# TorchIO-project/torchio

Measured on NVIDIA H100. Metric: augmented voxels/sec on 256^3 fp32 Compose pipeline, higher is better.
Workload: dtype f32

## Files before the change

### include/tio_b200.h

```cpp
#ifndef TIO_B200_H
#define TIO_B200_H

#include <stddef.h>
#include <stdint.h>

#ifdef __cplusplus
extern "C" {
#endif

#define TIO_ABI_VERSION 2

enum tio_dtype {
  TIO_F32 = 0,
  TIO_U8 = 1,
  TIO_I8 = 2,
  TIO_I16 = 3,
  TIO_I32 = 4,
  TIO_I64 = 5,
  TIO_F16 = 6,
  TIO_BF16 = 7,
  TIO_F64 = 8
};

enum tio_interp { TIO_NEAREST = 0, TIO_LINEAR = 1, TIO_LABEL_PV = 2 };
// ... 22 lines not shown

int tio_crop_patches(const void* src, void* dst, int elem_bytes, int C, int I, int J, int K,
                     int n, const int32_t* corners, int pi, int pj, int pk, void* stream);

int tio_remap(const void* src, void* dst, int elem_bytes, int B, int C, int I, int J, int K,
              int OI, int OJ, int OK, int off_i, int off_j, int off_k, int mode,
              const void* fill, const uint8_t* flip, void* stream);

int tio_upload(const void* host_pinned, void* dst_device, size_t bytes, void* stream);

int tio_min_sample0(const float* src, int C, int64_t n, float* fill, void* stream);

int tio_blur(const float* src, float* dst, float* scratch,
             int B, int C, int I, int J, int K,
             const float* taps, const int32_t* radius, int R, int axes_mask,
             const uint8_t* identity, void* stream);

size_t tio_mt19937_table_bytes(void);
int tio_mt19937_build_table(void* host_blob, size_t bytes);
size_t tio_randn_mt19937_workspace_bytes(uint64_t offset, uint64_t n);
int tio_randn_mt19937(uint64_t seed, uint64_t offset, uint64_t n, float* z,
                      const void* table, void* workspace, size_t workspace_bytes,
                      void* stream);

int tio_moments(const float* src, const uint8_t* mask, int64_t n, double* out3, void* stream);
size_t tio_quantiles_workspace_bytes(void);
int tio_quantiles(const float* src, const uint8_t* mask, int64_t n, const double* q_host, int m,
                  float* values, double* weights, double* count, void* workspace,
                  size_t workspace_bytes, void* stream);
int tio_rescale(const float* src, float* dst, int B, int64_t per_elem, float lo, float hi,
                const float* sub, const float* div, const float* mul, const float* add,
                const uint8_t* keep, int flags, void* stream);

size_t tio_quantiles_batched_workspace_bytes(int B, int m);
int tio_quantiles_batched(const void* src, int dtype, const uint8_t* mask, int B, int64_t per_elem,
                          const double* q_host, int m, float* values, double* weights, double* count,
                          uint8_t* has_nan, void* workspace, size_t workspace_bytes, void* stream);
int tio_histogram_tables(const float* values, const double* weights, const uint8_t* has_nan,
                         const float* landmarks, int B, int m, float* tables, void* stream);
int tio_histogram_map(const void* src, void* dst, int dtype, int B, int64_t per_elem,
                      const float* tables, int m, void* stream);

int tio_intensity_fused(const float* src, float* dst, float* scratch,
                        int B, int C, int I, int J, int K,
                        const float* coarse, int si, int sj, int sk,
                        const uint8_t* bias_identity, int bias_divide,
// ... 51 lines not shown
```

### torchio_b200/_native.py

```python

from __future__ import annotations

import ctypes
from ctypes import c_char_p, c_float, c_int, c_int64, c_size_t, c_uint64, c_void_p
from pathlib import Path

LIB_PATH = Path(__file__).resolve().parent / "csrc" / "libtio_b200.so"

_SIGNATURES = {
    "tio_abi_version": [],
    "tio_resample": [c_void_p, c_void_p, c_int] + [c_int] * 8
    + [c_void_p, c_void_p, c_void_p] + [c_int] * 3
    + [c_void_p, c_void_p, c_int, c_int, c_void_p, c_int, c_void_p, c_size_t, c_void_p],
    "tio_resample_workspace_bytes": [c_int, c_int, c_int, c_int],
    "tio_min_sample0": [c_void_p, c_int, c_int64, c_void_p, c_void_p],
    "tio_upload": [c_void_p, c_void_p, c_size_t, c_void_p],
    "tio_remap": [c_void_p, c_void_p, c_int] + [c_int] * 8 + [c_int] * 3 + [c_int, c_void_p, c_void_p, c_void_p],
    "tio_crop_patches": [c_void_p, c_void_p, c_int] + [c_int] * 5 + [c_void_p, c_int, c_int, c_int, c_void_p],
    "tio_blur": [c_void_p, c_void_p, c_void_p] + [c_int] * 5
    + [c_void_p, c_void_p, c_int, c_int, c_void_p, c_void_p],
    "tio_moments": [c_void_p, c_void_p, c_int64, c_void_p, c_void_p],
    "tio_quantiles_workspace_bytes": [],
    "tio_quantiles": [c_void_p, c_void_p, c_int64, c_void_p, c_int, c_void_p, c_void_p, c_void_p, c_void_p,
                      c_size_t, c_void_p],
    "tio_quantiles_batched_workspace_bytes": [c_int, c_int],
    "tio_quantiles_batched": [c_void_p, c_int, c_void_p, c_int, c_int64, c_void_p, c_int, c_void_p, c_void_p,
                              c_void_p, c_void_p, c_void_p, c_size_t, c_void_p],
    "tio_histogram_tables": [c_void_p, c_void_p, c_void_p, c_void_p, c_int, c_int, c_void_p, c_void_p],
    "tio_histogram_map": [c_void_p, c_void_p, c_int, c_int, c_int64, c_void_p, c_int, c_void_p],
    "tio_rescale": [c_void_p, c_void_p, c_int, c_int64, c_float, c_float, c_void_p, c_void_p, c_void_p, c_void_p,
                    c_void_p, c_int, c_void_p],
    "tio_onehot": [c_void_p, c_int, c_int, c_int64, c_void_p, c_int, c_void_p, c_void_p],
    "tio_label_argmax": [c_void_p, c_int, c_int, c_int64, c_void_p, c_float, c_void_p, c_int, c_void_p],
    "tio_mt19937_table_bytes": [],
    "tio_mt19937_build_table": [c_void_p, c_size_t],
    "tio_randn_mt19937_workspace_bytes": [c_uint64, c_uint64],
    "tio_randn_mt19937": [c_uint64, c_uint64, c_uint64, c_void_p, c_void_p, c_void_p, c_size_t,
                          c_void_p],
    "tio_intensity_fused": [c_void_p, c_void_p, c_void_p] + [c_int] * 5
    + [c_void_p, c_int, c_int, c_int, c_void_p, c_int]
    + [c_void_p, c_void_p, c_int, c_int]
    + [c_void_p] * 5 + [c_uint64, c_int, c_int, c_void_p, c_void_p],
    "tio_labels_to_image": [c_void_p, c_int, c_int, c_int, c_int64, c_void_p, c_int, c_void_p, c_void_p, c_void_p,
                            c_uint64, c_int, c_void_p, c_void_p],
    "tio_label_lut": [c_void_p, c_void_p, c_int, c_int64, c_void_p, c_void_p, c_int, c_int, c_void_p],
    "tio_label_contour": [c_void_p, c_int, c_int, c_int, c_int, c_int, c_void_p, c_void_p],
    "tio_onehot_classes": [c_void_p, c_int, c_int, c_int, c_int64, c_int, c_void_p, c_void_p],
    "tio_label_range": [c_void_p, c_int, c_int, c_int, c_int64, c_void_p, c_void_p],
    "tio_channel_argmax": [c_void_p, c_int, c_int, c_int, c_int64, c_void_p, c_void_p],
    "tio_interpolate": [c_void_p, c_void_p, c_int, c_int, c_int, c_int, c_int, c_int, c_int, c_int, c_void_p,
                        c_void_p, c_int, c_void_p],
    "tio_axis_resample": [c_void_p, c_void_p, c_int, c_int, c_int, c_int, c_int, c_int, c_void_p, c_void_p,
                          c_void_p, c_void_p, c_int, c_int, c_void_p],
    "tio_clamp": [c_void_p, c_void_p, c_int, c_int, c_int64, c_void_p, c_void_p, c_void_p],
    "tio_mask": [c_void_p, c_int, c_int, c_void_p, c_int, c_void_p, c_int, c_void_p, c_int, c_int, c_int, c_int64,
                 c_void_p, c_void_p],
    "tio_swap_patches": [c_void_p] + [c_int] * 9 + [c_void_p, c_int, c_int, c_void_p, c_void_p, c_void_p],
    "tio_components": [c_void_p] + [c_int] * 6 + [c_void_p, c_int, c_int64, c_int, c_int] + [c_void_p] * 4,
    "tio_component_roots": [c_void_p, c_int, c_int, c_int64] + [c_void_p] * 4,
    "tio_keep_largest": [c_void_p, c_int, c_int, c_int64, c_int, c_void_p, c_int, c_int64, c_int] + [c_void_p] * 5,
}
# ... 35 lines not shown
```

### torchio_b200/csrc/build.py

```python

from __future__ import annotations

import os
import subprocess
import sys
from concurrent.futures import ThreadPoolExecutor
from pathlib import Path

HERE = Path(__file__).resolve().parent
ROOT = HERE.parent.parent
SOURCES = ["error.cu", "resample.cu", "resample_tile.cu", "resample_fast.cu", "upload.cu", "fused_intensity.cu",
           "mt19937_jump.cpp", "mt19937.cu", "patches.cu", "stats.cu", "labels.cu", "labels_to_image.cu",
           "label_maps.cu", "interpolate.cu", "clamp_mask_swap.cu", "components.cu"]
HEADERS = [HERE / "common.cuh", HERE / "resample_common.cuh", HERE / "resample_tile.cuh", HERE / "tma.cuh",
           HERE / "mt19937_layout.h", HERE / "label_lookup.cuh", HERE / "image_dtype.cuh",
           ROOT / "include" / "tio_b200.h",
           Path(__file__).resolve()]
OBJ = HERE / "_obj"
OUT = HERE / "libtio_b200.so"

ARCH = ["-gencode", "arch=compute_90a,code=sm_90a"]
NVCC_FLAGS = [
    *ARCH,
    "-O3", "-std=c++17", "-lineinfo",
    "-Xcompiler", "-fPIC",
    "-Xptxas", "-v",
]


def needs_build() -> bool:
    if not OUT.exists():
        return True
    newest = max(p.stat().st_mtime for p in [*(HERE / s for s in SOURCES), *HEADERS])
    return OUT.stat().st_mtime < newest


def _compile(source: str) -> tuple[str, int, str]:
    src = HERE / source
    obj = OBJ / (Path(source).stem + ".o")
# ... 38 lines not shown
```

### torchio_b200/csrc/fused_intensity.cu

```cuda
#include "common.cuh"
#include "tma.cuh"

namespace tio {

__device__ __forceinline__ float rician(float x, float n1, float n2) {
  float s = __fadd_rn(x, n1);
  return sqrtf(__fadd_rn(__fmul_rn(s, s), __fmul_rn(n2, n2)));
}


__device__ __forceinline__ uint4 philox4x32_10(uint4 ctr, uint2 key) {
  const uint32_t M0 = 0xD2511F53u, M1 = 0xCD9E8D57u, W0 = 0x9E3779B9u, W1 = 0xBB67AE85u;
#pragma unroll
  for (int r = 0; r < 7; ++r) {
    uint32_t hi0 = __umulhi(M0, ctr.x), lo0 = M0 * ctr.x;
    uint32_t hi1 = __umulhi(M1, ctr.z), lo1 = M1 * ctr.z;
    ctr = make_uint4(hi1 ^ ctr.y ^ key.x, lo1, hi0 ^ ctr.w ^ key.y, lo0);
    key.x += W0;
    key.y += W1;
  }
  return ctr;
}

__device__ __forceinline__ void box_muller(uint32_t a, uint32_t b, float& n0, float& n1) {
  float u1 = ((float)(a >> 8) + 0.5f) * (1.0f / 16777216.0f);
  float u2 = ((float)(b >> 8)) * (1.0f / 16777216.0f);
  float rad;
  asm("sqrt.approx.ftz.f32 %0, %1;" : "=f"(rad) : "f"(-2.0f * __logf(u1)));
  float s, c;
  __sincosf(6.283185307179586f * u2, &s, &c);
  n0 = rad * c;
  n1 = rad * s;
}


__device__ __forceinline__ float abs_pow(float ax, float g) {
  float l, p;
  asm("lg2.approx.f32 %0, %1;" : "=f"(l) : "f"(ax));
  asm("ex2.approx.f32 %0, %1;" : "=f"(p) : "f"(__fmul_rn(g, l)));
  return p;
}

__device__ __forceinline__ float signed_pow(float x, float gam) {
  if (gam == 1.0f) return x;
  float ax = fabsf(x);
  float p = abs_pow(ax, gam);
  p = ax == 0.0f ? 0.0f : p;
  return x < 0.0f ? -p : p;
}

constexpr int A_TJ = 32;
constexpr int A_TK = 64;
constexpr int A_PLANES = 16;

struct BiasArgs {
  const float* coarse;
  const uint8_t* identity;
  int si, sj, sk;
  float sc_i, sc_j, sc_k;
  int divide;
};

struct BlurArgs {
  const float* taps;
  const int32_t* radius;
  int R;
};

struct NoiseArgs {
  const float* mean;
  const float* std;
  const uint8_t* keep;
// ... 192 lines not shown
    for (int o = 0; o < 4; ++o) acc[o] = __fmaf_rn(tk[F_R + t], win[F_HK + o + t], acc[o]);
  return make_float4(acc[0], acc[1], acc[2], acc[3]);
}

template <int RJ>
__device__ __forceinline__ void jconv8(const float* __restrict__ Bw, const int jy, const int kx,
                                       const float* tj, float* acc) {
  float win[8 + 2 * RJ];
#pragma unroll
  for (int w = 0; w < 8 + 2 * RJ; ++w) win[w] = Bw[(F_R - RJ + jy + w) * A_TK + kx];
  if (RJ == 0) {
#pragma unroll
    for (int o = 0; o < 8; ++o) acc[o] = win[o];
    return;
  }
#pragma unroll
  for (int o = 0; o < 8; ++o) acc[o] = 0.0f;
#pragma unroll
  for (int t = -RJ; t <= RJ; ++t)
#pragma unroll
    for (int o = 0; o < 8; ++o) acc[o] = __fmaf_rn(tj[F_R + t], win[o + t + RJ], acc[o]);
}

__device__ __forceinline__ float signed_pow_pos(float x, float g) {
  const float p = abs_pow(fabsf(x), g);
  return x < 0.0f ? -p : p;
}

template <bool HAS_EPI>
__global__ void __launch_bounds__(256, 3)
jk6_kernel(const __grid_constant__ CUtensorMap tmap, float* __restrict__ dst, int B, int C, int I,
           int J, int K, BlurArgs bl, NoiseArgs nz, const float* __restrict__ gamma) {
  extern __shared__ __align__(128) float smem[];
  float* Abuf = smem;
  float* Bbuf = smem + 2 * F_ABUF;
  float* taps_s = Bbuf + 2 * F_BBUF;
  uint64_t* bars = reinterpret_cast<uint64_t*>(taps_s + 32);

  const int tiles_i = (I + A_PLANES - 1) / A_PLANES;
  const int bc = blockIdx.z / tiles_i;
  const int i_begin = (blockIdx.z % tiles_i) * A_PLANES;
  const int i_end = min(i_begin + A_PLANES, I);
  const int b = bc / C;
  const int j0 = blockIdx.y * A_TJ, k0 = blockIdx.x * A_TK;
  const int tid = threadIdx.x;
  const int64_t n = (int64_t)I * J * K;

  auto issue = [&](int i, int s) {
    const uint32_t bar = smem_u32(bars + s);
    mbar_expect_tx(bar, (uint32_t)(F_ABUF * sizeof(float)));
    tma_load_3d(smem_u32(Abuf + s * F_ABUF), &tmap, k0 - F_HK, j0 - F_R, bc * I + i, bar);
  };
  if (tid == 0) {
    mbar_init(smem_u32(bars + 0), 1);
    mbar_init(smem_u32(bars + 1), 1);
    mbar_fence_init();
    issue(i_begin, 0);
  }

  const int R = bl.R;
  const int rj = bl.radius[1 * B + b], rk = bl.radius[2 * B + b];
  const bool noise_on = HAS_EPI && nz.mode != 0 && (!nz.keep || nz.keep[b]);
  const float mu = (HAS_EPI && nz.mode) ? nz.mean[b] : 0.0f, sd = (HAS_EPI && nz.mode) ? nz.std[b] : 0.0f;
  const float gam = (HAS_EPI && gamma) ? gamma[b] : 1.0f;
  const int gamma_mode = !(HAS_EPI && gamma) || gam == 1.0f ? 0 : (gam > 0.0f ? 1 : 2);

  if (tid < 2 * (2 * F_R + 1)) {
    const int axis = tid < (2 * F_R + 1) ? 2 : 1;
    const int s = tid < (2 * F_R + 1) ? tid : tid - (2 * F_R + 1);
    const int off = s - F_R, rr = axis == 2 ? rk : rj;
    float v = 0.0f;
    if (rr > 0 && off >= -rr && off <= rr) v = bl.taps[((int64_t)axis * B + b) * (2 * R + 1) + R + off];
    taps_s[(axis == 2 ? 0 : 13) + s] = v;
  }
  __syncthreads();
  float tk[2 * F_R + 1], tj[2 * F_R + 1];
#pragma unroll
  for (int t = 0; t < 2 * F_R + 1; ++t) { tk[t] = taps_s[t]; tj[t] = taps_s[13 + t]; }

  const int row_lo = F_R - rj, row_hi = F_R + A_TJ + rj;
  const int rsrc_lo = max(0, F_R - j0), rsrc_hi = min(F_ROWS - 1, J - 1 - j0 + F_R);
  const int clo = max(0, F_HK - k0), chi = min(F_COLS - 1, K - 1 - k0 + F_HK);
  const bool kfix = (clo > F_HK - rk) || (chi < F_HK + A_TK + rk - 1);

  const int k4 = (tid & 15) * 4;
  const int kx = tid & 63, jy = (tid >> 6) * 8;
  const int k = k0 + kx;
  const int valid = (k < K) ? min(8, J - (j0 + jy)) : 0;
// ... 66 lines not shown
      default: jconv8<6>(Bw, jy, kx, tj, acc); break;
    }
    if (valid > 0) {
      if (HAS_EPI && noise_on) {
        if (nz.mode == 2) {
          const uint2 key = make_uint2((uint32_t)nz.philox_seed, (uint32_t)(nz.philox_seed >> 32));
#pragma unroll
          for (int h = 0; h < 2; ++h) {
            const uint64_t gidx = (uint64_t)(flat0 + (int64_t)(4 * h) * K);
            uint4 rr = philox4x32_10(make_uint4((uint32_t)gidx, (uint32_t)(gidx >> 32), 0u, 0x6a6bu), key);
            box_muller(rr.x, rr.y, z1[4 * h], z1[4 * h + 1]);
            box_muller(rr.z, rr.w, z1[4 * h + 2], z1[4 * h + 3]);
            if (nz.rician) {
              uint4 r2 = philox4x32_10(make_uint4((uint32_t)gidx, (uint32_t)(gidx >> 32), 1u, 0x6a6bu), key);
              box_muller(r2.x, r2.y, z2[4 * h], z2[4 * h + 1]);
              box_muller(r2.z, r2.w, z2[4 * h + 2], z2[4 * h + 3]);
            }
          }
        }
        if (nz.rician) {
#pragma unroll
          for (int o = 0; o < 8; ++o)
            acc[o] = rician(acc[o], __fadd_rn(mu, __fmul_rn(sd, z1[o])), __fadd_rn(mu, __fmul_rn(sd, z2[o])));
        } else {
#pragma unroll
          for (int o = 0; o < 8; ++o) acc[o] = __fadd_rn(acc[o], __fadd_rn(mu, __fmul_rn(sd, z1[o])));
        }
      }
      if (gamma_mode == 1) {
#pragma unroll
        for (int o = 0; o < 8; ++o) acc[o] = signed_pow_pos(acc[o], gam);
      } else if (gamma_mode == 2) {
#pragma unroll
        for (int o = 0; o < 8; ++o) acc[o] = signed_pow(acc[o], gam);
      }
      float* yp = dst + flat0;
      if (valid == 8) {
#pragma unroll
        for (int o = 0; o < 8; ++o, yp += K) *yp = acc[o];
      } else {
#pragma unroll
        for (int o = 0; o < 8; ++o, yp += K)
          if (o < valid) *yp = acc[o];
      }
    }
    __syncthreads();
  }
}

template <int V, bool HAS_BIAS>
__global__ void __launch_bounds__(256)
march_kernel(const float* __restrict__ src, float* __restrict__ dst, int B, int C, int I, int J,
             int K, BlurArgs bl, BiasArgs bi, NoiseArgs nz, const float* __restrict__ gamma) {
  extern __shared__ __align__(16) float smem[];
  const int bc = blockIdx.z;
  const int b = bc / C;
  const int tid = threadIdx.y * blockDim.x + threadIdx.x;
  const int k = (blockIdx.x * blockDim.x + threadIdx.x) * V;
// ... 175 lines not shown
  const int64_t n = (int64_t)I * J * K;
  const float* x = src + (int64_t)bc * n;
  float* y = dst + (int64_t)bc * n;

  const int r = bl.taps ? bl.radius[0 * B + b] : 0;
  float* tapi = smem;
  float* g = smem + 16;
  const int ns = HAS_BIAS ? bi.si * bi.sj * bi.sk : 0;
  const bool bias_on = HAS_BIAS && !(bi.identity && bi.identity[b]);
  if (tid < W) {
    const int off = tid - F_R;
    tapi[tid] = (r > 0 && off >= -r && off <= r) ? bl.taps[((int64_t)0 * B + b) * (2 * bl.R + 1) + bl.R + off] : 0.0f;
  }
  if (bias_on) {
    const float* gs = bi.coarse + (int64_t)bc * ns;
    for (int t = tid; t < ns; t += 256) g[t] = gs[t];
  }
  __syncthreads();
  if (k >= K || j >= J) return;

  const bool noise_on = EPI && nz.mode != 0 && (!nz.keep || nz.keep[b]);
  const float mu = (EPI && nz.mode) ? nz.mean[b] : 0.0f, sd = (EPI && nz.mode) ? nz.std[b] : 0.0f;
  const float gam = (EPI && gamma) ? gamma[b] : 1.0f;
  const int gamma_mode = !(EPI && gamma) || gam == 1.0f ? 0 : (gam > 0.0f ? 1 : 2);

  LerpAxis lj, lk[4];
  int o00[4], o01[4], o10[4], o11[4];
  int cur0 = -1, cur1 = -1;
  float r_lo[4], r_hi[4];
  if (bias_on) {
    lj = lerp_axis(bi.sc_j, bi.sj, j);
#pragma unroll
    for (int v = 0; v < 4; ++v) {
      lk[v] = lerp_axis(bi.sc_k, bi.sk, k + v);
      o00[v] = lj.i0 * bi.sk + lk[v].i0; o01[v] = lj.i0 * bi.sk + lk[v].i1;
      o10[v] = lj.i1 * bi.sk + lk[v].i0; o11[v] = lj.i1 * bi.sk + lk[v].i1;
    }
  }
  const int col = j * K + k;
  const int plane = J * K;

  float4* fifo = reinterpret_cast<float4*>(g + ((ns + 3) / 4) * 4) + tid;
  auto fifo_issue = [&](int pl) {
    if (pl < I) {
      const uint32_t sa = (uint32_t)__cvta_generic_to_shared(fifo + (pl & (M6_PF - 1)) * 256);
      asm volatile("cp.async.cg.shared.global [%0], [%1], 16;" ::"r"(sa), "l"(x + (int64_t)pl * plane + col) : "memory");
    }
// ... 11 lines not shown
      const LerpAxis li = lerp_axis(bi.sc_i, bi.si, i);
      if (li.i0 != cur0 || li.i1 != cur1) {
        const float* p0 = g + (li.i0 * bi.sj) * bi.sk;
        const float* p1 = g + (li.i1 * bi.sj) * bi.sk;
#pragma unroll
        for (int v = 0; v < 4; ++v) {
          const float a0 = lerp2(lk[v].l0, p0[o00[v]], lk[v].l1, p0[o01[v]]);
          const float a1 = lerp2(lk[v].l0, p0[o10[v]], lk[v].l1, p0[o11[v]]);
          r_lo[v] = lerp2(lj.l0, a0, lj.l1, a1);
          const float b0 = lerp2(lk[v].l0, p1[o00[v]], lk[v].l1, p1[o01[v]]);
          const float b1 = lerp2(lk[v].l0, p1[o10[v]], lk[v].l1, p1[o11[v]]);
          r_hi[v] = lerp2(lj.l0, b0, lj.l1, b1);
        }
        cur0 = li.i0; cur1 = li.i1;
      }
#pragma unroll
      for (int v = 0; v < 4; ++v) {
        const float f = expf(lerp2(li.l0, r_lo[v], li.l1, r_hi[v]));
        out[v] = bi.divide ? __fdiv_rn(out[v], f) : __fmul_rn(out[v], f);
      }
    }
  };

  auto finish = [&](int i, float* v) {
    const int64_t o = (int64_t)i * plane + col;
    if (EPI) {
      if (noise_on) {
        const int64_t flat = (int64_t)bc * n + o;
        float z1[4], z2[4];
        if (nz.mode == 1) {
          const float4 t = __ldcs((const float4*)(nz.z + flat));
          z1[0] = t.x; z1[1] = t.y; z1[2] = t.z; z1[3] = t.w;
          if (nz.rician) {
            const float4 u = __ldcs((const float4*)(nz.z2 + flat));
            z2[0] = u.x; z2[1] = u.y; z2[2] = u.z; z2[3] = u.w;
          }
        } else {
          const uint2 key = make_uint2((uint32_t)nz.philox_seed, (uint32_t)(nz.philox_seed >> 32));
          const uint64_t gidx = (uint64_t)(flat / 4);
          uint4 rr = philox4x32_10(make_uint4((uint32_t)gidx, (uint32_t)(gidx >> 32), 0u, 0x5eedu), key);
          box_muller(rr.x, rr.y, z1[0], z1[1]);
          box_muller(rr.z, rr.w, z1[2], z1[3]);
          if (nz.rician) {
            uint4 r2 = philox4x32_10(make_uint4((uint32_t)gidx, (uint32_t)(gidx >> 32), 1u, 0x5eedu), key);
            box_muller(r2.x, r2.y, z2[0], z2[1]);
            box_muller(r2.z, r2.w, z2[2], z2[3]);
          }
        }
#pragma unroll
        for (int q = 0; q < 4; ++q) {
          const float n1 = __fadd_rn(mu, __fmul_rn(sd, z1[q]));
          if (nz.rician) v[q] = rician(v[q], n1, __fadd_rn(mu, __fmul_rn(sd, z2[q])));
          else v[q] = __fadd_rn(v[q], n1);
        }
      }
      if (gamma_mode == 1) {
#pragma unroll
        for (int q = 0; q < 4; ++q) v[q] = signed_pow_pos(v[q], gam);
      } else if (gamma_mode == 2) {
#pragma unroll
        for (int q = 0; q < 4; ++q) v[q] = signed_pow(v[q], gam);
      }
    }
    *(float4*)(y + o) = make_float4(v[0], v[1], v[2], v[3]);
  };

  if (r == 0) {
    for (int i = 0; i < I; ++i) {
      float v[4];
      load_plane(i, v);
      finish(i, v);
    }
    return;
  }

  float tp[W];
#pragma unroll
  for (int t = 0; t < W; ++t) tp[t] = tapi[t];
  float ring[W][4];
  {
    float first[4];
    load_plane(0, first);
#pragma unroll
    for (int sl = 0; sl < W; ++sl)
#pragma unroll
// ... 295 lines not shown
```

### torchio_b200/csrc/mt19937.cu

```cuda
#include "common.cuh"
#include "mt19937_layout.h"

namespace tio {

constexpr int MT_N = 624, MT_M = 397, MT_DEG = 19937;
constexpr int MT_SEQ = MT_DEG + MT_N;
constexpr int MT_OFFS = (MT_SEQ + 7) / 4 * 4;

__device__ __forceinline__ uint32_t mt_twist(uint32_t a, uint32_t b, uint32_t c) {
  const uint32_t y = (a & 0x80000000u) | (b & 0x7fffffffu);
  return c ^ (y >> 1) ^ ((y & 1u) ? 0x9908b0dfu : 0u);
}

__device__ __forceinline__ uint32_t mt_temper(uint32_t y) {
  y ^= y >> 11;
  y ^= (y << 7) & 0x9d2c5680u;
  y ^= (y << 15) & 0xefc60000u;
  y ^= y >> 18;
  return y;
}

__global__ void mt_seed_kernel(uint32_t seed, uint32_t* __restrict__ states) {
  if (threadIdx.x == 0) {
    uint32_t v = seed;
// ... 90 lines not shown
  float sn, cs;
  sincos_0_2pi(theta, sn, cs);
  zc = radius * cs;
  zs = radius * sn;
}

template <int ID, int COUNT>
__device__ __forceinline__ void mt_bar_sync() {
  asm volatile("bar.sync %0, %1;" ::"n"(ID), "n"(COUNT) : "memory");
}
template <int ID, int COUNT>
__device__ __forceinline__ void mt_bar_arrive() {
  asm volatile("bar.arrive %0, %1;" ::"n"(ID), "n"(COUNT) : "memory");
}

constexpr int MT_ROUND = 4;
constexpr int MT_RING = 2 * MT_ROUND;
constexpr int MT_ITEMS = MT_ROUND * MT_N / 8;
constexpr int MT_PRODUCERS = 256;
constexpr int MT_CONSUMERS = (MT_ITEMS + 31) / 32 * 32;
constexpr int MT_THREADS = MT_PRODUCERS + MT_CONSUMERS;
constexpr int MT_BAR_PROD = 1, MT_BAR_FULL = 2, MT_BAR_EMPTY = 4;

__global__ void __launch_bounds__(MT_THREADS, 2)
mt_normal_kernel(const uint32_t* __restrict__ states, int q_first, unsigned long long L,
                 unsigned long long offset, unsigned long long n, float* __restrict__ z) {
  __shared__ __align__(16) uint32_t ring[MT_RING * MT_N];
  const int tid = threadIdx.x;
  const int q = q_first + blockIdx.x;
  const unsigned long long seg_begin = (unsigned long long)q * L;
  const unsigned long long lo = max(seg_begin, offset);
  const unsigned long long hi = min(seg_begin + L, offset + n);
  if (lo >= hi) return;
  const int lo_rel = (int)(lo - seg_begin), hi_rel = (int)(hi - seg_begin);
  const int rounds = ((hi_rel + MT_N - 1) / MT_N + MT_ROUND - 1) / MT_ROUND;
  if (tid < MT_PRODUCERS) {
    constexpr int W = MT_N - MT_M;
    const uint32_t* w = states + (size_t)q * MT_N;
    uint32_t* start = ring + (MT_RING - 1) * MT_N;
    for (int t = tid; t < MT_N; t += MT_PRODUCERS) start[t] = w[t];
    mt_bar_sync<MT_BAR_PROD, MT_PRODUCERS>();
    for (int r = 0; r < rounds; ++r) {
      if (r >= 2) {
        if (r & 1) mt_bar_sync<MT_BAR_EMPTY + 1, MT_THREADS>();
        else mt_bar_sync<MT_BAR_EMPTY, MT_THREADS>();
      }
      for (int i = 0; i < MT_ROUND; ++i) {
        const int b = r * MT_ROUND + i;
        const uint32_t* cur = ring + ((b + MT_RING - 1) % MT_RING) * MT_N;
        uint32_t* nxt = ring + (b % MT_RING) * MT_N;
        if (tid < W) nxt[tid] = mt_twist(cur[tid], cur[tid + 1], cur[tid + MT_M]);
        mt_bar_sync<MT_BAR_PROD, MT_PRODUCERS>();
        if (tid < W) nxt[W + tid] = mt_twist(cur[W + tid], cur[W + tid + 1], nxt[tid]);
        mt_bar_sync<MT_BAR_PROD, MT_PRODUCERS>();
        if (tid < MT_N - 2 * W) {
          const int k = 2 * W + tid;
          const uint32_t c = (k + 1 < MT_N) ? cur[k + 1] : nxt[0];
          nxt[k] = mt_twist(cur[k], c, nxt[k - W]);
        }
        mt_bar_sync<MT_BAR_PROD, MT_PRODUCERS>();
      }
      if (r & 1) mt_bar_arrive<MT_BAR_FULL + 1, MT_THREADS>();
      else mt_bar_arrive<MT_BAR_FULL, MT_THREADS>();
    }
  } else {
    const int c = tid - MT_PRODUCERS;
    const int blk = c / (MT_N / 8), item = c % (MT_N / 8);
    const int word = 16 * (item >> 1) + 4 * (item & 1);
    const long long seg_to_z = (long long)seg_begin - (long long)offset;
    const bool vec = ((reinterpret_cast<uintptr_t>(z) & 15) == 0);
    for (int r = 0; r < rounds; ++r) {
      if (r & 1) mt_bar_sync<MT_BAR_FULL + 1, MT_THREADS>();
      else mt_bar_sync<MT_BAR_FULL, MT_THREADS>();
      const int b = r * MT_ROUND + blk;
      const int group = b * MT_N + (word & ~15);
      if (c < MT_ITEMS && group >= lo_rel && group < hi_rel) {
        const uint32_t* x = ring + (b % MT_RING) * MT_N + word;
        const uint4 a = *reinterpret_cast<const uint4*>(x);
        const uint4 s = *reinterpret_cast<const uint4*>(x + 8);
        float4 zc, zs;
        mt_box_muller(a.x, s.x, zc.x, zs.x);
        mt_box_muller(a.y, s.y, zc.y, zs.y);
        mt_box_muller(a.z, s.z, zc.z, zs.z);
        mt_box_muller(a.w, s.w, zc.w, zs.w);
        float* zp = z + (seg_to_z + b * MT_N + word);
        if (vec) {
          *reinterpret_cast<float4*>(zp) = zc;
          *reinterpret_cast<float4*>(zp + 8) = zs;
        } else {
          zp[0] = zc.x; zp[1] = zc.y; zp[2] = zc.z; zp[3] = zc.w;
          zp[8] = zs.x; zp[9] = zs.y; zp[10] = zs.z; zp[11] = zs.w;
        }
      }
      if (r + 2 < rounds) {
        if (r & 1) mt_bar_arrive<MT_BAR_EMPTY + 1, MT_THREADS>();
        else mt_bar_arrive<MT_BAR_EMPTY, MT_THREADS>();
      }
    }
  }
}

}

using namespace tio;

constexpr uint64_t MT_L = 1ull << tio_mt::kLog2L;

extern "C" size_t tio_randn_mt19937_workspace_bytes(uint64_t offset, uint64_t n) {
  const uint64_t q_hi = (offset + n + MT_L - 1) / MT_L;
  return (size_t)(q_hi + tio_mt::kS1) * MT_N * 4;
}

extern "C" int tio_randn_mt19937(uint64_t seed, uint64_t offset, uint64_t n, float* z,
                                 const void* table, void* workspace, size_t workspace_bytes,
                                 void* stream) {
  TIO_CHECK_ARG(z && table && workspace, "tio_randn_mt19937: null pointer");
  TIO_CHECK_ARG(n >= 16 && (n % 16) == 0 && (offset % 16) == 0,
                "tio_randn_mt19937: n and offset must be multiples of 16 (n >= 16)");
  const int S2 = tio_mt::kS2, S1 = tio_mt::kS1, stride = tio_mt::kStride;
  const uint64_t q_lo = offset / MT_L, q_hi = (offset + n + MT_L - 1) / MT_L;
  TIO_CHECK_ARG(q_hi <= (uint64_t)S1 * S2, "tio_randn_mt19937: stream position beyond %d segments", S1 * S2);
  TIO_CHECK_ARG(workspace_bytes >= tio_randn_mt19937_workspace_bytes(offset, n),
                "tio_randn_mt19937: workspace too small");
  cudaStream_t st = (cudaStream_t)stream;
  uint32_t* states = (uint32_t*)workspace;
  const uint16_t* polys = (const uint16_t*)((const char*)table + tio_mt::kHeaderBytes);
  mt_seed_kernel<<<1, 32, 0, st>>>((uint32_t)seed, states);
  const size_t jump_smem = (size_t)(MT_OFFS + 2048) * 4;
  cudaFuncSetAttribute(mt_jump_kernel, cudaFuncAttributeMaxDynamicSharedMemorySize, (int)jump_smem);
  const int m_lo = (int)(q_lo / S2), m_hi = (int)((q_hi - 1) / S2);
  const int m_first = m_lo > 1 ? m_lo : 1;
  if (m_hi >= m_first) {
    constexpr int kCoarseParts = 8;
    const size_t pitch = (size_t)S2 * MT_N * 4;
    cudaMemset2DAsync(states + (size_t)m_first * S2 * MT_N, pitch, 0, MT_N * 4, m_hi - m_first + 1, st);
    mt_jump_kernel<<<(m_hi - m_first + 1) * kCoarseParts, 640, jump_smem, st>>>(states, polys, stride, m_first,
                                                                             S2, 0, kCoarseParts);
  }
  mt_jump_kernel<<<(unsigned)(q_hi - q_lo), 640, jump_smem, st>>>(states, polys, stride, (int)q_lo, S2, 1, 1);
  mt_normal_kernel<<<(unsigned)(q_hi - q_lo), MT_THREADS, 0, st>>>(states, (int)q_lo, MT_L, offset, n, z);
  TIO_CHECK_LAUNCH();
  return 0;
}
```

### torchio_b200/ops.py

```python

from __future__ import annotations

import os
import threading

import numpy as np
import torch
from torch import Tensor

from . import _native, tables

DTYPE_CODES = {
    torch.float32: 0, torch.uint8: 1, torch.int8: 2,
    torch.int16: 3, torch.int32: 4, torch.int64: 5,
}
NEAREST, LINEAR, LABEL_PV = 0, 1, 2
FLAG_PASSTHROUGH, FLAG_ELASTIC = 1, 2

_counter = threading.local()


def launches() -> int:
    return getattr(_counter, "n", 0)

# ... 460 lines not shown
            table = _mt_device_tables.get(key)
            if table is None:
                table = mt19937_host_table().to(device)
                torch.cuda.synchronize(device)
                _mt_device_tables[key] = table
    return table


def randn_mt19937(seed: int, offset: int, n: int, device, out: Tensor | None = None) -> Tensor:
    device = torch.device(device)
    if n < 16 or n % 16 or offset % 16 or offset + n > MT_MAX_WORDS:
        raise ValueError("randn_mt19937: offset and n must be multiples of 16, n >= 16,"
                         " offset + n <= 2**31")
    z = torch.empty(n, dtype=torch.float32, device=device) if out is None else out
    lib = _native.lib()
    ws_bytes = lib.tio_randn_mt19937_workspace_bytes(offset, n)
    workspace = torch.empty(ws_bytes, dtype=torch.uint8, device=device)
    table = _mt_table(device)
    with torch.cuda.device(device):
        _native.call("tio_randn_mt19937", int(seed) & 0xFFFFFFFF, offset, n, _ptr(z), _ptr(table),
                     _ptr(workspace), ws_bytes, torch.cuda.current_stream(device).cuda_stream)
    _count(4)
    return z



_cuda_rng_lock = threading.Lock()


def labels_to_image(labels: Tensor, label_values, means, stds, draw=None) -> Tensor:
    if labels.dtype not in DTYPE_CODES:
        raise TypeError(f"labels_to_image: unsupported label dtype {labels.dtype}")
    if labels.ndim != 5:
        raise ValueError(f"labels_to_image expects (B, C, I, J, K), got {tuple(labels.shape)}")
    b, c = int(labels.shape[0]), int(labels.shape[1])
    vox = int(np.prod(labels.shape[2:]))
    numel = b * vox
    tables.check_randn_numel(numel)
    _require_cuda(labels, "labels_to_image")
    if torch.cuda.is_current_stream_capturing():
        raise RuntimeError("labels_to_image: CUDA-graph capture is not supported (the generator offsets are"
                           " reserved on the host)")
    values = np.ascontiguousarray(np.asarray(label_values, dtype=np.int64).reshape(-1))
    n = int(values.shape[0])
    if n and np.any(np.diff(values) <= 0):
        raise ValueError("labels_to_image: label_values must be strictly ascending")
# ... 306 lines not shown
```

### torchio_b200/transforms/intensity.py

```python

from __future__ import annotations

import os
import warnings
from typing import Any

import numpy as np
import torch
from torch import Tensor

from .. import ops, tables
from ..data import ImagesBatch, LabelMap, ScalarImage, SubjectsBatch
from ..params import to_nonneg_range, to_range
from .base import IntensityTransform, Transform, chunk_info, staged_derived


def _as_f32(data: Tensor) -> Tensor:
    return data if data.dtype == torch.float32 else data.float()




class BiasField(IntensityTransform):
    def __init__(self, *, std=0.5, scale: float = 0.025, **kwargs: Any) -> None:
# ... 183 lines not shown
        mean = self._mask_identity(self.mean.sample_1d(n), keep, identity=0.0)
        std = self._mask_identity(self.std.sample_1d(n), keep, identity=0.0)
        params = {
            "mean": self._serialize_param(mean), "std": self._serialize_param(std),
            "seed": seed, "rician": self.rician,
        }
        self._tag_batched(params, batch, n, keep, ["mean", "std"])
        return params

    def apply_transform(self, batch: SubjectsBatch, params: dict[str, Any]) -> SubjectsBatch:
        run_stages(self._get_images(batch), [_noise_stage_factory(params)])
        return batch


def _noise_stage_factory(params):
    mode = _noise_mode()
    generator = torch.Generator(device="cpu")
    generator.manual_seed(params["seed"])
    rician = bool(params.get("rician", False))
    keep = params.get("_keep")

    consumed = [0]

    def draw(shape, device):
        n = int(np.prod(shape))
        info = chunk_info()
        if info is None:
            start, n_full = consumed[0], n
        else:
            per = n // shape[0]
            start, n_full = consumed[0] + per * info.b0, per * info.total
        on_device = (not ragged[0] and n >= 16 and n % 16 == 0 and start % 16 == 0
                     and n_full % 16 == 0 and start + n <= ops.MT_MAX_WORDS
                     and device.type == "cuda")
        if info is not None and not on_device:
            raise RuntimeError("Noise: this batch cannot be streamed in slices (ragged normal stream)")
        if n_full < 16 or n_full % 16:
            ragged[0] = True
        consumed[0] += n_full + (16 if (n_full >= 16 and n_full % 16) else 0)
        if on_device:
            return ops.randn_mt19937(params["seed"], start, n, device).view(shape), None
        if host_state[0] != start:
            skip = start - host_state[0]
            if skip % 16 == 0 and skip >= 16:
                torch.randn(skip, generator=generator)
            else:
                raise RuntimeError("Noise: cannot realign the host generator (ragged stream)")
        pin = torch.cuda.is_available()
        z = torch.empty(shape, dtype=torch.float32, pin_memory=pin)
        torch.randn(shape, generator=generator, out=z)
        host_state[0] = consumed[0]
        return None, z

    host_state = [0]
    ragged = [False]

    def stage(ib, index):
        shape = ib.data.shape
        b = shape[0]
        out = {
            "mean": tables.per_element_vector(params["mean"], b),
            "std": tables.per_element_vector(params["std"], b),
            "keep": None if keep is None else np.asarray(keep, dtype=np.uint8),
            "rician": rician,
        }
        if mode == "philox":
            out["noise_mode"] = 2
            out["philox_seed"] = (int(params["seed"]) << 8) | (index & 0xFF)
            return out
        out["noise_mode"] = 1
        z_dev, z_host = draw(shape, ib.data.device)
        out["z" if z_dev is not None else "z_host"] = z_dev if z_dev is not None else z_host
        if rician:
            z_dev, z_host = draw(shape, ib.data.device)
            out["z2" if z_dev is not None else "z2_host"] = z_dev if z_dev is not None else z_host
        return out

    return stage




class Gamma(IntensityTransform):
    def __init__(self, *, log_gamma=0.0, **kwargs: Any) -> None:
        super().__init__(**kwargs)
        self.log_gamma = to_range(log_gamma)
        self._warn_if_noop(is_noop=self.log_gamma.is_constant(0.0), hint="log_gamma=(-0.3, 0.3)")

    @property
    def supports_per_instance_params(self) -> bool:
        return True

    @property
    def supports_per_instance_p(self) -> bool:
        return True

    def supports_chunks(self, batch: SubjectsBatch) -> bool:
        return True
# ... 360 lines not shown
_TABLE_KEYS = ("coarse", "bias_identity", "taps", "radius", "mean", "std", "keep", "gamma")


def run_stages(images, stage_builders) -> None:
    for index, ib in enumerate(images.values()):
        kwargs: dict[str, Any] = {}
        for build in stage_builders:
            stage = build(ib, index)
            if stage:
                kwargs.update(stage)
        if not kwargs:
            continue
        data = ib.data
        device = data.device
        uploaded = ops.upload(device, *[kwargs.get(k) for k in _TABLE_KEYS])
        for key, value in zip(_TABLE_KEYS, uploaded, strict=True):
            if key in kwargs:
                kwargs[key] = value
        z_host, z2_host = kwargs.pop("z_host", None), kwargs.pop("z2_host", None)
        if z_host is not None:
            kwargs["z"] = z_host.to(device, non_blocking=True)
        if z2_host is not None:
            kwargs["z2"] = z2_host.to(device, non_blocking=True)
        out = ops.intensity_fused(_as_f32(data), **kwargs)
        promotes = ("gamma" in kwargs or "mean" in kwargs) and data.dtype != torch.float64
        ib.data = out if promotes or out.dtype == data.dtype else out.to(data.dtype)
```

Measured before the change: 49.40 billion.

## Fuse MT19937 Gaussian noise and gamma into the RNG kernel epilogue

```diff
diff --git a/include/tio_b200.h b/include/tio_b200.h
--- a/include/tio_b200.h
+++ b/include/tio_b200.h
@@ -68,6 +68,11 @@
 int tio_randn_mt19937(uint64_t seed, uint64_t offset, uint64_t n, float* z,
                       const void* table, void* workspace, size_t workspace_bytes,
                       void* stream);
+
+int tio_noise_mt19937(uint64_t seed, uint64_t offset, uint64_t n, const float* src, float* dst,
+                      uint64_t elem_words, const float* mean, const float* std,
+                      const uint8_t* keep, const float* gamma, const void* table,
+                      void* workspace, size_t workspace_bytes, void* stream);
 
 int tio_moments(const float* src, const uint8_t* mask, int64_t n, double* out3, void* stream);
 size_t tio_quantiles_workspace_bytes(void);
diff --git a/torchio_b200/_native.py b/torchio_b200/_native.py
--- a/torchio_b200/_native.py
+++ b/torchio_b200/_native.py
@@ -37,6 +37,8 @@
     "tio_randn_mt19937_workspace_bytes": [c_uint64, c_uint64],
     "tio_randn_mt19937": [c_uint64, c_uint64, c_uint64, c_void_p, c_void_p, c_void_p, c_size_t,
                           c_void_p],
+    "tio_noise_mt19937": [c_uint64, c_uint64, c_uint64, c_void_p, c_void_p, c_uint64, c_void_p, c_void_p,
+                          c_void_p, c_void_p, c_void_p, c_void_p, c_size_t, c_void_p],
     "tio_intensity_fused": [c_void_p, c_void_p, c_void_p] + [c_int] * 5
     + [c_void_p, c_int, c_int, c_int, c_void_p, c_int]
     + [c_void_p, c_void_p, c_int, c_int]
diff --git a/torchio_b200/csrc/build.py b/torchio_b200/csrc/build.py
--- a/torchio_b200/csrc/build.py
+++ b/torchio_b200/csrc/build.py
@@ -14,7 +14,7 @@
            "label_maps.cu", "interpolate.cu", "clamp_mask_swap.cu", "components.cu"]
 HEADERS = [HERE / "common.cuh", HERE / "resample_common.cuh", HERE / "resample_tile.cuh", HERE / "tma.cuh",
            HERE / "mt19937_layout.h", HERE / "label_lookup.cuh", HERE / "image_dtype.cuh",
-           ROOT / "include" / "tio_b200.h",
+           HERE / "intensity_epilogue.cuh", ROOT / "include" / "tio_b200.h",
            Path(__file__).resolve()]
 OBJ = HERE / "_obj"
 OUT = HERE / "libtio_b200.so"
diff --git a/torchio_b200/csrc/fused_intensity.cu b/torchio_b200/csrc/fused_intensity.cu
--- a/torchio_b200/csrc/fused_intensity.cu
+++ b/torchio_b200/csrc/fused_intensity.cu
@@ -1,4 +1,5 @@
 #include "common.cuh"
+#include "intensity_epilogue.cuh"
 #include "tma.cuh"
 
 namespace tio {
@@ -33,21 +34,6 @@
   n1 = rad * s;
 }
 
-
-__device__ __forceinline__ float abs_pow(float ax, float g) {
-  float l, p;
-  asm("lg2.approx.f32 %0, %1;" : "=f"(l) : "f"(ax));
-  asm("ex2.approx.f32 %0, %1;" : "=f"(p) : "f"(__fmul_rn(g, l)));
-  return p;
-}
-
-__device__ __forceinline__ float signed_pow(float x, float gam) {
-  if (gam == 1.0f) return x;
-  float ax = fabsf(x);
-  float p = abs_pow(ax, gam);
-  p = ax == 0.0f ? 0.0f : p;
-  return x < 0.0f ? -p : p;
-}
 
 constexpr int A_TJ = 32;
 constexpr int A_TK = 64;
@@ -286,11 +272,6 @@
     for (int o = 0; o < 8; ++o) acc[o] = __fmaf_rn(tj[F_R + t], win[o + t + RJ], acc[o]);
 }
 
-__device__ __forceinline__ float signed_pow_pos(float x, float g) {
-  const float p = abs_pow(fabsf(x), g);
-  return x < 0.0f ? -p : p;
-}
-
 template <bool HAS_EPI>
 __global__ void __launch_bounds__(256, 3)
 jk6_kernel(const __grid_constant__ CUtensorMap tmap, float* __restrict__ dst, int B, int C, int I,
@@ -327,7 +308,7 @@
   const bool noise_on = HAS_EPI && nz.mode != 0 && (!nz.keep || nz.keep[b]);
   const float mu = (HAS_EPI && nz.mode) ? nz.mean[b] : 0.0f, sd = (HAS_EPI && nz.mode) ? nz.std[b] : 0.0f;
   const float gam = (HAS_EPI && gamma) ? gamma[b] : 1.0f;
-  const int gamma_mode = !(HAS_EPI && gamma) || gam == 1.0f ? 0 : (gam > 0.0f ? 1 : 2);
+  const int gamma_mode = gamma_mode_of(HAS_EPI ? gamma : nullptr, gam);
 
   if (tid < 2 * (2 * F_R + 1)) {
     const int axis = tid < (2 * F_R + 1) ? 2 : 1;
@@ -440,18 +421,9 @@
 #pragma unroll
           for (int o = 0; o < 8; ++o)
             acc[o] = rician(acc[o], __fadd_rn(mu, __fmul_rn(sd, z1[o])), __fadd_rn(mu, __fmul_rn(sd, z2[o])));
-        } else {
-#pragma unroll
-          for (int o = 0; o < 8; ++o) acc[o] = __fadd_rn(acc[o], __fadd_rn(mu, __fmul_rn(sd, z1[o])));
-        }
-      }
-      if (gamma_mode == 1) {
-#pragma unroll
-        for (int o = 0; o < 8; ++o) acc[o] = signed_pow_pos(acc[o], gam);
-      } else if (gamma_mode == 2) {
-#pragma unroll
-        for (int o = 0; o < 8; ++o) acc[o] = signed_pow(acc[o], gam);
-      }
+        }
+      }
+      noise_gamma(acc, z1, HAS_EPI && noise_on && !nz.rician, mu, sd, gamma_mode, gam);
       float* yp = dst + flat0;
       if (valid == 8) {
 #pragma unroll
@@ -673,7 +645,7 @@
   const bool noise_on = EPI && nz.mode != 0 && (!nz.keep || nz.keep[b]);
   const float mu = (EPI && nz.mode) ? nz.mean[b] : 0.0f, sd = (EPI && nz.mode) ? nz.std[b] : 0.0f;
   const float gam = (EPI && gamma) ? gamma[b] : 1.0f;
-  const int gamma_mode = !(EPI && gamma) || gam == 1.0f ? 0 : (gam > 0.0f ? 1 : 2);
+  const int gamma_mode = gamma_mode_of(EPI ? gamma : nullptr, gam);
 
   LerpAxis lj, lk[4];
   int o00[4], o01[4], o10[4], o11[4];
@@ -731,12 +703,12 @@
     }
   };
 
-  auto finish = [&](int i, float* v) {
+  auto finish = [&](int i, float (&v)[4]) {
     const int64_t o = (int64_t)i * plane + col;
     if (EPI) {
+      float z1[4], z2[4];
       if (noise_on) {
         const int64_t flat = (int64_t)bc * n + o;
-        float z1[4], z2[4];
         if (nz.mode == 1) {
           const float4 t = __ldcs((const float4*)(nz.z + flat));
           z1[0] = t.x; z1[1] = t.y; z1[2] = t.z; z1[3] = t.w;
@@ -756,20 +728,13 @@
             box_muller(r2.z, r2.w, z2[2], z2[3]);
           }
         }
-#pragma unroll
-        for (int q = 0; q < 4; ++q) {
-          const float n1 = __fadd_rn(mu, __fmul_rn(sd, z1[q]));
-          if (nz.rician) v[q] = rician(v[q], n1, __fadd_rn(mu, __fmul_rn(sd, z2[q])));
-          else v[q] = __fadd_rn(v[q], n1);
-        }
-      }
-      if (gamma_mode == 1) {
-#pragma unroll
-        for (int q = 0; q < 4; ++q) v[q] = signed_pow_pos(v[q], gam);
-      } else if (gamma_mode == 2) {
-#pragma unroll
-        for (int q = 0; q < 4; ++q) v[q] = signed_pow(v[q], gam);
-      }
+        if (nz.rician) {
+#pragma unroll
+          for (int q = 0; q < 4; ++q)
+            v[q] = rician(v[q], __fadd_rn(mu, __fmul_rn(sd, z1[q])), __fadd_rn(mu, __fmul_rn(sd, z2[q])));
+        }
+      }
+      noise_gamma(v, z1, noise_on && !nz.rician, mu, sd, gamma_mode, gam);
     }
     *(float4*)(y + o) = make_float4(v[0], v[1], v[2], v[3]);
   };
diff --git a/torchio_b200/csrc/intensity_epilogue.cuh b/torchio_b200/csrc/intensity_epilogue.cuh
--- /dev/null
+++ b/torchio_b200/csrc/intensity_epilogue.cuh
@@ -0,0 +1,45 @@
+#pragma once
+
+namespace tio {
+
+__device__ __forceinline__ float abs_pow(float ax, float g) {
+  float l, p;
+  asm("lg2.approx.f32 %0, %1;" : "=f"(l) : "f"(ax));
+  asm("ex2.approx.f32 %0, %1;" : "=f"(p) : "f"(__fmul_rn(g, l)));
+  return p;
+}
+
+__device__ __forceinline__ float signed_pow(float x, float gam) {
+  if (gam == 1.0f) return x;
+  float ax = fabsf(x);
+  float p = abs_pow(ax, gam);
+  p = ax == 0.0f ? 0.0f : p;
+  return x < 0.0f ? -p : p;
+}
+
+__device__ __forceinline__ float signed_pow_pos(float x, float g) {
+  const float p = abs_pow(fabsf(x), g);
+  return x < 0.0f ? -p : p;
+}
+
+__device__ __forceinline__ int gamma_mode_of(const float* gamma, float g) {
+  return !gamma || g == 1.0f ? 0 : (g > 0.0f ? 1 : 2);
+}
+
+template <int N>
+__device__ __forceinline__ void noise_gamma(float (&v)[N], const float (&z)[N], bool noise_on, float mu,
+                                            float sd, int gamma_mode, float g) {
+  if (noise_on) {
+#pragma unroll
+    for (int i = 0; i < N; ++i) v[i] = __fadd_rn(v[i], __fadd_rn(mu, __fmul_rn(sd, z[i])));
+  }
+  if (gamma_mode == 1) {
+#pragma unroll
+    for (int i = 0; i < N; ++i) v[i] = signed_pow_pos(v[i], g);
+  } else if (gamma_mode == 2) {
+#pragma unroll
+    for (int i = 0; i < N; ++i) v[i] = signed_pow(v[i], g);
+  }
+}
+
+}
diff --git a/torchio_b200/csrc/mt19937.cu b/torchio_b200/csrc/mt19937.cu
--- a/torchio_b200/csrc/mt19937.cu
+++ b/torchio_b200/csrc/mt19937.cu
@@ -1,4 +1,5 @@
 #include "common.cuh"
+#include "intensity_epilogue.cuh"
 #include "mt19937_layout.h"
 
 namespace tio {
@@ -136,10 +137,27 @@
 constexpr int MT_THREADS = MT_PRODUCERS + MT_CONSUMERS;
 constexpr int MT_BAR_PROD = 1, MT_BAR_FULL = 2, MT_BAR_EMPTY = 4;
 
+struct MtApply {
+  const float* src;
+  float* dst;
+  uint32_t elem_words;
+  const float* mean;
+  const float* std;
+  const uint8_t* keep;
+  const float* gamma;
+};
+
+__device__ __forceinline__ void mt_cp_async16(void* smem, const void* gmem) {
+  const uint32_t sa = (uint32_t)__cvta_generic_to_shared(smem);
+  asm volatile("cp.async.cg.shared.global [%0], [%1], 16;" ::"r"(sa), "l"(gmem) : "memory");
+}
+
+template <bool APPLY>
 __global__ void __launch_bounds__(MT_THREADS, 2)
 mt_normal_kernel(const uint32_t* __restrict__ states, int q_first, unsigned long long L,
-                 unsigned long long offset, unsigned long long n, float* __restrict__ z) {
+                 unsigned long long offset, unsigned long long n, float* __restrict__ z, MtApply ap) {
   __shared__ __align__(16) uint32_t ring[MT_RING * MT_N];
+  __shared__ __align__(16) float4 staged[APPLY ? 2 * 2 * MT_CONSUMERS : 1];
   const int tid = threadIdx.x;
   const int q = q_first + blockIdx.x;
   const unsigned long long seg_begin = (unsigned long long)q * L;
@@ -182,13 +200,52 @@
     const int blk = c / (MT_N / 8), item = c % (MT_N / 8);
     const int word = 16 * (item >> 1) + 4 * (item & 1);
     const long long seg_to_z = (long long)seg_begin - (long long)offset;
-    const bool vec = ((reinterpret_cast<uintptr_t>(z) & 15) == 0);
+    constexpr int ROUND_WORDS = MT_ROUND * MT_N;
+    const int group0 = blk * MT_N + (word & ~15);
+    const uint32_t position0 = (uint32_t)(seg_to_z + group0) + (word & 15);
+    auto active = [&](int r) {
+      const int group = group0 + r * ROUND_WORDS;
+      return c < MT_ITEMS && group >= lo_rel && group < hi_rel;
+    };
+    auto position = [&](int r) { return position0 + (uint32_t)(r * ROUND_WORDS); };
+    const bool vec = APPLY ? ((reinterpret_cast<uintptr_t>(ap.src) | reinterpret_cast<uintptr_t>(ap.dst)) & 15) == 0
+                           : (reinterpret_cast<uintptr_t>(z) & 15) == 0;
+    auto prefetch = [&](int r) {
+      if (r < rounds && active(r)) {
+        const float* s = ap.src + position(r);
+        float4* d = staged + (r & 1) * 2 * MT_CONSUMERS + c;
+        mt_cp_async16(d, s);
+        mt_cp_async16(d + MT_CONSUMERS, s + 8);
+      }
+      asm volatile("cp.async.commit_group;" ::: "memory");
+    };
+    if (APPLY && vec) prefetch(0);
+    uint32_t e_end = 0;
+    bool noise_on = false;
+    float mu = 0.0f, sd = 0.0f, g = 1.0f;
+    int gm = 0;
     for (int r = 0; r < rounds; ++r) {
+      const bool on = active(r);
+      uint32_t t = 0;
+      if (APPLY) {
+        if (vec) prefetch(r + 1);
+        if (on) {
+          t = position(r);
+          if (t >= e_end) {
+            const uint32_t e = t / ap.elem_words;
+            e_end = (e + 1) * ap.elem_words;
+            noise_on = !ap.keep || ap.keep[e];
+            mu = ap.mean[e];
+            sd = ap.std[e];
+            g = ap.gamma ? ap.gamma[e] : 1.0f;
+            gm = gamma_mode_of(ap.gamma, g);
+          }
+        }
+      }
       if (r & 1) mt_bar_sync<MT_BAR_FULL + 1, MT_THREADS>();
       else mt_bar_sync<MT_BAR_FULL, MT_THREADS>();
-      const int b = r * MT_ROUND + blk;
-      const int group = b * MT_N + (word & ~15);
-      if (c < MT_ITEMS && group >= lo_rel && group < hi_rel) {
+      if (on) {
+        const int b = r * MT_ROUND + blk;
         const uint32_t* x = ring + (b % MT_RING) * MT_N + word;
         const uint4 a = *reinterpret_cast<const uint4*>(x);
         const uint4 s = *reinterpret_cast<const uint4*>(x + 8);
@@ -197,7 +254,25 @@
         mt_box_muller(a.y, s.y, zc.y, zs.y);
         mt_box_muller(a.z, s.z, zc.z, zs.z);
         mt_box_muller(a.w, s.w, zc.w, zs.w);
-        float* zp = z + (seg_to_z + b * MT_N + word);
+        if (APPLY) {
+          float4 va, vb;
+          if (vec) {
+            asm volatile("cp.async.wait_group 1;" ::: "memory");
+            const float4* sp = staged + (r & 1) * 2 * MT_CONSUMERS + c;
+            va = sp[0];
+            vb = sp[MT_CONSUMERS];
+          } else {
+            const float* sp = ap.src + t;
+            va = make_float4(sp[0], sp[1], sp[2], sp[3]);
+            vb = make_float4(sp[8], sp[9], sp[10], sp[11]);
+          }
+          float v[8] = {va.x, va.y, va.z, va.w, vb.x, vb.y, vb.z, vb.w};
+          const float zz[8] = {zc.x, zc.y, zc.z, zc.w, zs.x, zs.y, zs.z, zs.w};
+          noise_gamma(v, zz, noise_on, mu, sd, gm, g);
+          zc = make_float4(v[0], v[1], v[2], v[3]);
+          zs = make_float4(v[4], v[5], v[6], v[7]);
+        }
+        float* zp = (APPLY ? ap.dst : z) + position(r);
         if (vec) {
           *reinterpret_cast<float4*>(zp) = zc;
           *reinterpret_cast<float4*>(zp + 8) = zs;
@@ -225,18 +300,17 @@
   return (size_t)(q_hi + tio_mt::kS1) * MT_N * 4;
 }
 
-extern "C" int tio_randn_mt19937(uint64_t seed, uint64_t offset, uint64_t n, float* z,
-                                 const void* table, void* workspace, size_t workspace_bytes,
-                                 void* stream) {
-  TIO_CHECK_ARG(z && table && workspace, "tio_randn_mt19937: null pointer");
+static int mt_start_states(uint64_t seed, uint64_t offset, uint64_t n, const void* table, void* workspace,
+                           size_t workspace_bytes, cudaStream_t st, const char* who, uint64_t& q_lo,
+                           uint64_t& q_hi) {
+  TIO_CHECK_ARG(table && workspace, "%s: null pointer", who);
   TIO_CHECK_ARG(n >= 16 && (n % 16) == 0 && (offset % 16) == 0,
-                "tio_randn_mt19937: n and offset must be multiples of 16 (n >= 16)");
+                "%s: n and offset must be multiples of 16 (n >= 16)", who);
   const int S2 = tio_mt::kS2, S1 = tio_mt::kS1, stride = tio_mt::kStride;
-  const uint64_t q_lo = offset / MT_L, q_hi = (offset + n + MT_L - 1) / MT_L;
-  TIO_CHECK_ARG(q_hi <= (uint64_t)S1 * S2, "tio_randn_mt19937: stream position beyond %d segments", S1 * S2);
-  TIO_CHECK_ARG(workspace_bytes >= tio_randn_mt19937_workspace_bytes(offset, n),
-                "tio_randn_mt19937: workspace too small");
-  cudaStream_t st = (cudaStream_t)stream;
+  q_lo = offset / MT_L;
+  q_hi = (offset + n + MT_L - 1) / MT_L;
+  TIO_CHECK_ARG(q_hi <= (uint64_t)S1 * S2, "%s: stream position beyond %d segments", who, S1 * S2);
+  TIO_CHECK_ARG(workspace_bytes >= tio_randn_mt19937_workspace_bytes(offset, n), "%s: workspace too small", who);
   uint32_t* states = (uint32_t*)workspace;
   const uint16_t* polys = (const uint16_t*)((const char*)table + tio_mt::kHeaderBytes);
   mt_seed_kernel<<<1, 32, 0, st>>>((uint32_t)seed, states);
@@ -252,7 +326,37 @@
                                                                              S2, 0, kCoarseParts);
   }
   mt_jump_kernel<<<(unsigned)(q_hi - q_lo), 640, jump_smem, st>>>(states, polys, stride, (int)q_lo, S2, 1, 1);
-  mt_normal_kernel<<<(unsigned)(q_hi - q_lo), MT_THREADS, 0, st>>>(states, (int)q_lo, MT_L, offset, n, z);
+  return 0;
+}
+
+extern "C" int tio_randn_mt19937(uint64_t seed, uint64_t offset, uint64_t n, float* z,
+                                 const void* table, void* workspace, size_t workspace_bytes,
+                                 void* stream) {
+  TIO_CHECK_ARG(z, "tio_randn_mt19937: null pointer");
+  cudaStream_t st = (cudaStream_t)stream;
+  uint64_t q_lo, q_hi;
+  if (mt_start_states(seed, offset, n, table, workspace, workspace_bytes, st, "tio_randn_mt19937", q_lo, q_hi))
+    return 1;
+  mt_normal_kernel<false><<<(unsigned)(q_hi - q_lo), MT_THREADS, 0, st>>>((const uint32_t*)workspace, (int)q_lo,
+                                                                           MT_L, offset, n, z, MtApply{});
   TIO_CHECK_LAUNCH();
   return 0;
 }
+
+extern "C" int tio_noise_mt19937(uint64_t seed, uint64_t offset, uint64_t n, const float* src, float* dst,
+                                 uint64_t elem_words, const float* mean, const float* std,
+                                 const uint8_t* keep, const float* gamma, const void* table, void* workspace,
+                                 size_t workspace_bytes, void* stream) {
+  TIO_CHECK_ARG(src && dst && mean && std, "tio_noise_mt19937: null pointer");
+  TIO_CHECK_ARG(elem_words >= 16 && elem_words % 16 == 0 && n % elem_words == 0,
+                "tio_noise_mt19937: elem_words must be a multiple of 16 that divides n");
+  cudaStream_t st = (cudaStream_t)stream;
+  uint64_t q_lo, q_hi;
+  if (mt_start_states(seed, offset, n, table, workspace, workspace_bytes, st, "tio_noise_mt19937", q_lo, q_hi))
+    return 1;
+  const MtApply ap{src, dst, (uint32_t)elem_words, mean, std, keep, gamma};
+  mt_normal_kernel<true><<<(unsigned)(q_hi - q_lo), MT_THREADS, 0, st>>>((const uint32_t*)workspace, (int)q_lo,
+                                                                          MT_L, offset, n, nullptr, ap);
+  TIO_CHECK_LAUNCH();
+  return 0;
+}
diff --git a/torchio_b200/ops.py b/torchio_b200/ops.py
--- a/torchio_b200/ops.py
+++ b/torchio_b200/ops.py
@@ -506,6 +506,33 @@
                      _ptr(workspace), ws_bytes, torch.cuda.current_stream(device).cuda_stream)
     _count(4)
     return z
+
+
+def noise_mt19937(src: Tensor, seed: int, offset: int, *, mean: Tensor, std: Tensor, keep: Tensor | None = None,
+                  gamma: Tensor | None = None, out: Tensor | None = None) -> Tensor:
+    _require_cuda(src, "noise_mt19937")
+    if src.dtype != torch.float32:
+        raise ValueError("noise_mt19937: src must be float32")
+    src = src.contiguous()
+    n = src.numel()
+    elem = n // src.shape[0] if src.dim() and src.shape[0] else 0
+    if elem < 16 or elem % 16 or offset % 16 or offset + n > MT_MAX_WORDS:
+        raise ValueError("noise_mt19937: voxels per batch element and offset must be multiples of 16,"
+                         " offset + numel <= 2**31")
+    dst = torch.empty_like(src) if out is None else out
+    if dst.shape != src.shape or dst.dtype != src.dtype or not dst.is_contiguous() or dst.device != src.device:
+        raise ValueError("noise_mt19937: out must be a contiguous float32 tensor shaped like src")
+    device = src.device
+    lib = _native.lib()
+    ws_bytes = lib.tio_randn_mt19937_workspace_bytes(offset, n)
+    workspace = torch.empty(ws_bytes, dtype=torch.uint8, device=device)
+    table = _mt_table(device)
+    with torch.cuda.device(device):
+        _native.call("tio_noise_mt19937", int(seed) & 0xFFFFFFFF, offset, n, _ptr(src), _ptr(dst), elem,
+                     _ptr(mean), _ptr(std), _ptr(keep), _ptr(gamma), _ptr(table), _ptr(workspace), ws_bytes,
+                     _stream(src))
+    _count(4)
+    return dst
 
 
 
diff --git a/torchio_b200/transforms/intensity.py b/torchio_b200/transforms/intensity.py
--- a/torchio_b200/transforms/intensity.py
+++ b/torchio_b200/transforms/intensity.py
@@ -229,7 +229,7 @@
 
     consumed = [0]
 
-    def draw(shape, device):
+    def draw(shape, device, key, apply=False):
         n = int(np.prod(shape))
         info = chunk_info()
         if info is None:
@@ -246,7 +246,9 @@
             ragged[0] = True
         consumed[0] += n_full + (16 if (n_full >= 16 and n_full % 16) else 0)
         if on_device:
-            return ops.randn_mt19937(params["seed"], start, n, device).view(shape), None
+            if apply and (n // shape[0]) % 16 == 0:
+                return {"z_stream": (params["seed"], start)}
+            return {key: ops.randn_mt19937(params["seed"], start, n, device).view(shape)}
         if host_state[0] != start:
             skip = start - host_state[0]
             if skip % 16 == 0 and skip >= 16:
@@ -257,7 +259,7 @@
         z = torch.empty(shape, dtype=torch.float32, pin_memory=pin)
         torch.randn(shape, generator=generator, out=z)
         host_state[0] = consumed[0]
-        return None, z
+        return {key + "_host": z}
 
     host_state = [0]
     ragged = [False]
@@ -276,11 +278,9 @@
             out["philox_seed"] = (int(params["seed"]) << 8) | (index & 0xFF)
             return out
         out["noise_mode"] = 1
-        z_dev, z_host = draw(shape, ib.data.device)
-        out["z" if z_dev is not None else "z_host"] = z_dev if z_dev is not None else z_host
+        out.update(draw(shape, ib.data.device, "z", apply=not rician))
         if rician:
-            z_dev, z_host = draw(shape, ib.data.device)
-            out["z2" if z_dev is not None else "z2_host"] = z_dev if z_dev is not None else z_host
+            out.update(draw(shape, ib.data.device, "z2"))
         return out
 
     return stage
@@ -687,6 +687,20 @@
             kwargs["z"] = z_host.to(device, non_blocking=True)
         if z2_host is not None:
             kwargs["z2"] = z2_host.to(device, non_blocking=True)
-        out = ops.intensity_fused(_as_f32(data), **kwargs)
         promotes = ("gamma" in kwargs or "mean" in kwargs) and data.dtype != torch.float64
+        z_stream = kwargs.pop("z_stream", None)
+        if z_stream is None:
+            out = ops.intensity_fused(_as_f32(data), **kwargs)
+        else:
+            out = _fused_then_noise(_as_f32(data), kwargs, *z_stream)
         ib.data = out if promotes or out.dtype == data.dtype else out.to(data.dtype)
+
+
+def _fused_then_noise(src, kwargs, seed, start):
+    tail = {key: kwargs.pop(key, None) for key in ("mean", "std", "keep", "gamma")}
+    kwargs.pop("noise_mode")
+    kwargs.pop("rician")
+    if not kwargs:
+        return ops.noise_mt19937(src, seed, start, **tail)
+    out = ops.intensity_fused(src, **kwargs)
+    return ops.noise_mt19937(out, seed, start, out=out, **tail)
```

Result: faster. 50.33 billion (median of 6 runs) (+1.9%).
